# irmen/synthesizer

Hardware: AMD Instinct MI355X
Metric: Msamples/sec mixed to stereo bus, 1024-voice additive @48kHz (higher is better)
Workload: dtype f64

## Files before the change

### synthesizer_amd/csrc/osc_bank.hip

```cpp
#include "osc_host.hpp"
#include <new>
#include <stdlib.h>
#include <math.h>

namespace {

__global__ void k_prepare(BankPtrs B, uint32_t first, uint32_t nvoices, uint64_t start, uint32_t nframes,
                          VoiceLaunch* __restrict__ out, VoiceFM* __restrict__ out_fm) {
    uint32_t vi = blockIdx.x * blockDim.x + threadIdx.x;
    PrepInfo info;
    if (vi < nvoices) prepare_voice(B, first, vi, start, nframes, out, out_fm, info);
}

__global__ __launch_bounds__(64) void k_prepare_chunks(BankPtrs B, LaunchSet S, uint32_t nvoices, uint64_t start, uint32_t nframes) {
    prepare_chunk(B, S, blockIdx.x, nvoices, start, nframes);
}

__global__ __launch_bounds__(64) void k_prepare_segments(BankPtrs B, LaunchSet base, uint32_t nvoices, uint64_t start, uint32_t nframes,
                                                         uint32_t seg_frames) {
    const uint32_t s = blockIdx.y;
    const uint32_t first = s * seg_frames;
    const uint32_t n = nframes - first < seg_frames ? nframes - first : seg_frames;
    prepare_chunk(B, segment_set(base, s, nvoices), blockIdx.x, nvoices, start + first, n);
}

template <bool SLOPED>
__global__ __launch_bounds__(64) void k_prepare_segments_var(BankPtrs B, LaunchSet base, uint32_t nvoices, uint64_t start) {
    const uint32_t s = blockIdx.y;
    const uint32_t first = B.seg_first[s], n = B.seg_first[s + 1] - first;
    prepare_chunk<SLOPED>(B, segment_set(base, s, nvoices), blockIdx.x, nvoices, start + first, n);
}

__global__ __launch_bounds__(256) void k_prepare_tiles(BankPtrs B, TileSet T, uint32_t nvoices, uint64_t start, uint32_t nframes, uint32_t ntiles,
                                                       LaunchSet recs, uint32_t with_recs) {
    const uint32_t c = T.k0 * T.groups + blockIdx.x;
    if (c < (nvoices + 63) / 64)
        prepare_tiles_wave(B, T, nvoices, start, nframes, ntiles, c, blockIdx.y * 4 + (threadIdx.x >> 6), with_recs ? &recs : nullptr);
}

}

namespace shosc {

int launch_prepare_tiles(hipStream_t st, const BankPtrs& P, const TileSet& T, uint32_t nvoices, uint64_t start, uint32_t nframes, const LaunchSet* recs) {
    const uint32_t ntiles = sh::div_up(nframes, TILE_FRAMES);
    if (T.k1 == T.k0) return SH_OK;
    hipLaunchKernelGGL(k_prepare_tiles, dim3((T.k1 - T.k0) * T.groups, sh::div_up(ntiles, 4 * TILES_PER_WAVE)), dim3(256), 0, st, P, T, nvoices, start, nframes, ntiles,
                       recs ? *recs : LaunchSet(), recs ? 1u : 0u);
    SH_CHECK_LAUNCH("k_prepare_tiles");
    return SH_OK;
}

int grow_tile_set(sh::Pooled& block, TileSet& T, uint32_t& carved_tiles, uint32_t ntiles, uint32_t nvoices, uint32_t groups, uint32_t range_chunks, hipStream_t st) {
    const uint32_t mask_k = tile_mask_k(nvoices, groups);
    if (block.ptr && T.recs == (TileRec*)block.ptr && T.groups == groups && T.mask_k == mask_k && carved_tiles == ntiles && T.rec_chunks >= range_chunks) return SH_OK;
    uint32_t rec_chunks = ((range_chunks + range_chunks / 4 + 8) + 7) & ~7u;
    const uint32_t all_chunks = (nvoices + 63) / 64 + groups;
    if (rec_chunks > all_chunks) rec_chunks = all_chunks;
    if (rec_chunks < range_chunks) rec_chunks = range_chunks;
    const size_t slots = (size_t)rec_chunks * 64;
    const size_t b_recs = sizeof(TileRec) * ntiles * slots, b_mask = ((sizeof(uint64_t) * ntiles * groups * mask_k) + 255) & ~(size_t)255;
    int rc = sh::grow_pooled(block, b_recs + 2 * b_mask);
    if (rc) return rc;
    carved_tiles = ntiles;
    char* p = (char*)block.ptr;
    T.recs = (TileRec*)p; p += b_recs;
    T.lean = (uint64_t*)p; p += b_mask;
    T.gen = (uint64_t*)p;
    T.groups = groups;
    T.mask_k = mask_k;
    T.k0 = 0;
    T.k1 = 0;
    T.rec_chunks = rec_chunks;
    if (((nvoices + 63) / 64) != groups * mask_k) SH_HIP(hipMemsetAsync(T.lean, 0, 2 * b_mask, st));
    return SH_OK;
}

LaunchSet launch_set(const sh_bank* b, int k) {
    LaunchSet s;
    s.launch = b->d_launch_buf[k];
    s.fm = b->d_launch_fm_buf[k];
    s.fast = b->d_fast_buf[k];
    s.gen_idx = b->d_gen_idx_buf[k];
    s.counts = b->d_counts_buf[k];
    return s;
}

BankPtrs ptrs(const sh_bank* b) {
    BankPtrs p;
    p.voices = b->d_voices;
    p.segs = b->d_segs;
    p.coefs = b->d_coefs;
    p.partials = b->d_partials;
    p.hint = b->d_hint;
    p.lfo_hint = b->d_hint + b->nvoices;
    p.seg_rot = b->d_seg_rot;
    p.lfo_rot = b->d_lfo_rot;
    p.rows = b->launch_rows;
    p.row_stride = b->launch_row_stride;
    p.fm_row = b->d_fm_row;
    p.pwm_row = b->d_pwm_row;
    p.nseg = 0;
    for (int k = 0; k <= SEG_MAX; ++k) p.seg_first[k] = 0;
    p.gen_sub = 1;
    p.gen_scratch = nullptr;
    p.tiles = TileSet{nullptr, nullptr, nullptr, 0, 0, 0};
    p.next_tiles = p.tiles;
    p.next_tile_wgs = 0;
    p.next_ntiles = 0;
    p.polys = b->d_polys;
    p.chunk_span = b->d_chunk_span;
    return p;
}

template <typename T>
static int upload_array(T** dst, const T* src, size_t count, hipStream_t st) {
    *dst = nullptr;
    size_t bytes = (count ? count : 1) * sizeof(T);
    SH_HIP(hipMalloc((void**)dst, bytes));
    if (count) SH_HIP(hipMemcpyAsync(*dst, src, count * sizeof(T), hipMemcpyHostToDevice, st));
    return SH_OK;
}

std::vector<sh_bank*>& live_banks() {
    static std::vector<sh_bank*> v;
    return v;
}
// ... 391 lines not shown
```

### synthesizer_amd/csrc/osc_device.hpp

```cpp
#pragma once
#include "common.hpp"
#include "devmath.hpp"
#include "renderplan.hpp"
#include <type_traits>

namespace shosc {


constexpr uint32_t TILE_MAX_PIECES = 3;
struct alignas(64) TileRec {
    double t0, dt;
    double rc, rs;
    double ea0, ea1, eb0, eb1;
    double GL, GR;
    double tb[2], db[2];
    uint16_t split[2];
    uint16_t npieces;
    uint16_t corner;
    double pad_;
};
constexpr uint32_t TILE_WALK_PIECES = 16;
static_assert(sizeof(TileRec) == TILE_REC_BYTES && sizeof(TileRec) == 128 && offsetof(TileRec, GL) == 64 && offsetof(TileRec, tb) == 80 && offsetof(TileRec, split) == 112, "TileRec layout");
__device__ __forceinline__ double readlane_f64(double v, uint32_t src) {
    union { double d; int u[2]; } a, b;
    a.d = v;
    b.u[0] = __builtin_amdgcn_readlane(a.u[0], (int)src);
    b.u[1] = __builtin_amdgcn_readlane(a.u[1], (int)src);
    return b.d;
}
__device__ __forceinline__ uint32_t nth_set_bit(uint64_t m, uint32_t p) {
    uint32_t pos = 0;
#pragma unroll
    for (int w = 32; w >= 1; w >>= 1) {
        const uint64_t low = m & ((1ull << w) - 1ull);
        const uint32_t cnt = (uint32_t)__popcll(low);
        if (p >= cnt) { p -= cnt; m >>= w; pos += (uint32_t)w; } else { m = low; }
    }
    return pos;
}
struct TileTheta {
    double   lane_d, t0, dt, tb0, tb1, db0, db1;
    uint32_t lane, s1, s2;
    __device__ __forceinline__ double operator()(int j) const {
        const uint32_t i = lane + (uint32_t)j * 64u;
        const double dd = lane_d + (double)(j * 64);
        double t = fma(dd, dt, t0);
        if (i >= s1) t = fma(dd - (double)s1, db0, tb0);
        if (i >= s2) t = fma(dd - (double)s2, db1, tb1);
        return t;
    }
};
struct TileSet {
    TileRec*  recs;
    uint64_t* lean;
    uint64_t* gen;
    uint32_t  groups, mask_k;
    uint32_t  k0, k1;
    uint32_t  rec_chunks;
};
__host__ __device__ __forceinline__ uint32_t tile_mask_k(uint32_t nvoices, uint32_t groups) {
    const uint32_t nchunks = (nvoices + 63) / 64;
    return ((nchunks + groups - 1) / groups + 7) & ~7u;
}

struct BankPtrs {
    const sh_voice*   voices;
    const sh_segment* segs;
    const double*     coefs;
    const sh_partial* partials;
    uint32_t*         hint;
    uint32_t*         lfo_hint;
    const double2*    seg_rot;
    const double2*    lfo_rot;
    const double*     rows;
    size_t            row_stride;
    const int32_t*    fm_row;
    const int32_t*    pwm_row;
    uint32_t          nseg;
    uint32_t          seg_first[SEG_MAX + 1];
    uint32_t          gen_sub;
    double2*          gen_scratch;
    TileSet           tiles;
    const double*     polys;
    const uint64_t*   chunk_span;
    TileSet           next_tiles;
    uint32_t          next_tile_wgs, next_ntiles;
};

#define SH_CONST_AS __attribute__((address_space(4)))
template <typename T>
__device__ __forceinline__ const T SH_CONST_AS* as_const(const T* p) {
#pragma clang diagnostic push
#pragma clang diagnostic ignored "-Wold-style-cast"
    return (const T SH_CONST_AS*)p;
#pragma clang diagnostic pop
}

constexpr uint32_t FL_KIND = 0xF, FL_FM_SHIFT = 4, FL_FM = 0x30, FL_DENSE = 0x40, FL_ENV_UNIFORM = 0x80,
                   FL_POLY = 0x100, FL_FOLDED = 0x200, FL_FLIP = 0x400, FL_SILENT = 0x800, FL_ONSET = 0x1000;
constexpr uint32_t NO_TAIL = 0xFFFFFFFFu;
constexpr int NXP = 12;

struct alignas(16) VoiceLaunch {
    double   t_base, dt;
    uint32_t remain;
    uint32_t flags;
    const double* harm;
    double   amplitude, bias;
    double   gain_l, gain_r;
    double   g0u, slu;
    uint32_t harm_cnt;
// ... 1144 lines not shown
            }
            is_gen = !is_lean && !is_walk;
            if (is_walk) {
                rec_ea0 = wa0; rec_ea1 = wa1; rec_eb0 = wb0; rec_eb1 = wb1;
                rec_corner = w_corner;
            }
            if (is_lean) {
                rec_t0 = fma(dn0 - (double)p_n0, p_dt, p_t0);
                rec_extra = extra;
#pragma unroll
                for (uint32_t k = 0; k < 2; ++k) rec_split[k] = k < extra ? (uint16_t)((long long)starts[k] - n0) : (uint16_t)0xFFFFu;
            }
        }
        any_general = any_general || is_gen;
        if (sounds) { any_sound = true; last_piece = wb + r; }
        const uint64_t ml = __ballot(is_lean || is_walk), mg = __ballot(is_gen);
        const uint64_t mh = __ballot((is_lean || is_walk) && rec_kind == LEAN_HARM), mm = __ballot((is_lean || is_walk) && rec_kind == LEAN_FM);
        const uint32_t n_harm = (uint32_t)__popcll(mh), n_fm = (uint32_t)__popcll(mm);
        if (is_lean || is_walk) {
            const uint64_t below = (1ull << lane) - 1ull;
            const uint32_t pos = rec_kind == LEAN_HARM ? (uint32_t)__popcll(mh & below)
                               : rec_kind == LEAN_FM ? n_harm + (uint32_t)__popcll(mm & below)
                               : n_harm + n_fm + (uint32_t)__popcll(ml & ~mh & ~mm & below);
            TileRec* __restrict__ q = T.recs + (size_t)t * slots + (c - T.k0 * T.groups) * 64 + pos;
            const uint32_t corner = (rec_corner > 0 && rec_corner < TILE_FRAMES && !(rec_ea0 == rec_eb0 && rec_ea1 == rec_eb1)) ? rec_corner : 0u;
            if (!corner) { rec_eb0 = rec_ea0; rec_eb1 = rec_ea1; }
            double2* __restrict__ q2 = reinterpret_cast<double2*>(q);
            q2[0] = make_double2(rec_t0, win_pick<double>(w_dt, r, 0.0));
            double lfo_angle = 0.0;
            if (rec_kind == LEAN_FM)
                lfo_angle = lnp ? fma(dn0 - (double)ltab[2 * lp].n0 - 0.5, ltab[2 * lp].dt, ltab[2 * lp].t0) : fma(dn0 - 0.5, v.lfo_d, v.lfo_a);
            q2[1] = rec_kind == LEAN_FM ? make_double2(dn0, lfo_angle) : rot;
            q2[2] = make_double2(rec_ea0, rec_ea1);
            q2[3] = make_double2(rec_eb0, rec_eb1);
            q2[4] = make_double2(amp * bgl, amp * bgr);
            union { uint64_t u; double d; } walk_bits;
            walk_bits.u = (uint64_t)(off + wb + r) | ((uint64_t)(off + cnt) << 32);
            q2[5] = is_walk ? make_double2(dn0, walk_bits.d)
                            : make_double2(rec_extra > 0 ? win_pick<double>(w_t0, r + 1, 0.0) : 0.0, rec_extra > 1 ? win_pick<double>(w_t0, r + 2, 0.0) : 0.0);
            q2[6] = make_double2(rec_extra > 0 ? win_pick<double>(w_dt, r + 1, 0.0) : 0.0, rec_extra > 1 ? win_pick<double>(w_dt, r + 2, 0.0) : 0.0);
            union { uint16_t h[4]; double d; } tail;
            tail.h[0] = rec_split[0]; tail.h[1] = rec_split[1]; tail.h[2] = is_walk ? (uint16_t)0 : (uint16_t)(1 + rec_extra); tail.h[3] = (uint16_t)corner;
            union { uint32_t u[2]; double d; } kind_bits;
            kind_bits.u[0] = rec_kind | (rec_kind == LEAN_FM ? ((lnp ? off_c + 2 * lp : 0xFFFFFFu) << 8) : 0u);
            kind_bits.u[1] = lane | (lfo_split_rel << 8);
            q2[7] = make_double2(tail.d, kind_bits.d);
        }
        if (lane == 0) {
            const size_t at = ((size_t)t * T.groups + c % T.groups) * T.mask_k + c / T.groups;
            T.lean[at] = (uint64_t)(uint32_t)__popcll(ml) | ((uint64_t)n_harm << 32) | ((uint64_t)n_fm << 40);
            T.gen[at] = mg;
        }
    }
    if (recs) {
        if (valid && any_general) {
            PrepInfo info;
            prepare_voice<false>(B, 0u, vi, start, nframes, recs->launch, recs->fm, info);
        } else if (valid && any_sound) {
            B.hint[vi] = last_piece;
        }
        if (run == 0 && lane == 0) {
            recs->counts[4 * c] = 0; recs->counts[4 * c + 1] = 0; recs->counts[4 * c + 2] = 0; recs->counts[4 * c + 3] = 0;
        }
    }
}


}
```

### synthesizer_amd/csrc/osc_host.hpp

```cpp
#pragma once
#include "osc_device.hpp"
#include <vector>
#include <algorithm>

using namespace shosc;

struct sh_bank : shr::Facts {
    sh_voice*   d_voices = nullptr;
    sh_segment* d_segs = nullptr;
    double*     d_coefs = nullptr;
    sh_partial* d_partials = nullptr;
    static constexpr int NSETS = shosc::NSETS;
    VoiceLaunch* d_launch_buf[NSETS] = {};
    VoiceFM*    d_launch_fm_buf[NSETS] = {};
    FastRec*    d_fast_buf[NSETS] = {};
    uint32_t*   d_gen_idx_buf[NSETS] = {};
    uint32_t*   d_counts_buf[NSETS] = {};
    uint32_t*   d_hint = nullptr;
    static constexpr uint32_t SELF_TILES = shosc::SELF_TILES;
    uint32_t*   d_self() const { return d_hint + 2 * (size_t)nvoices; }
    bool        run_active = false;
    uint64_t    run_next_start = 0;
    uint32_t    run_nframes = 0, run_groups = 0, run_tile = 0, run_count = 0;
    sh::PendingCombine pending[2];
    int         npending = 0;
    sh::Pooled  parts[4];
    sh::Pooled  seg_block[2];
    LaunchSet   seg_set[2] = {};
    uint32_t    seg_cap[2] = {0, 0};
    sh::Pooled  seg_scratch[2];
    static constexpr int NTILESETS = 4;
    sh::Pooled  tile_block[NTILESETS];
    TileSet     tile_set[NTILESETS] = {};
    uint32_t    tile_carved[NTILESETS] = {0, 0, 0, 0};
    using TileSpec = shr::TileSetSpec;
    TileSpec    tile_spec[NTILESETS];
    uint32_t    tile_count = 0;
    struct Range { const char* lo; const char* hi; };
    Range       last_direct[3] = {};
    bool        overlaps_last_direct(const void* p, size_t bytes) const {
        const char* lo = (const char*)p;
        for (const Range& r : last_direct) if (r.lo && lo < r.hi && r.lo < lo + bytes) return true;
        return false;
    }
    int32_t*    d_fm_row = nullptr;
    int32_t*    d_pwm_row = nullptr;
    int32_t     fm_row_max = -1;
    bool        needs_rows = false;
    const double* launch_rows = nullptr;
    size_t      launch_row_stride = 0;
    sh::Pooled  gen_block;
    LaunchSet   gen_set = {};
    uint32_t    gen_segs = 0;
    double2*    d_seg_rot = nullptr;
    uint64_t*   d_chunk_span = nullptr;
    double*     d_polys = nullptr;
    double2*    d_lfo_rot = nullptr;
    VoiceLaunch* d_launch = nullptr;
    VoiceFM*    d_launch_fm = nullptr;
    int         cur = 0;
    int         last_target = -1;
    using Spec = shr::SetSpec;
    Spec        spec[NSETS];
    void        void_specs() { for (auto& q : spec) q.valid = false; last_target = -1; }
    bool        last_tiled = false;
    uint32_t    last_groups = 0;
    float2*     d_gains = nullptr;
    uint32_t    nsegs = 0, ncoefs = 0, npartials = 0;
    std::vector<sh_voice> h_voices;
};

namespace shosc {
LaunchSet launch_set(const sh_bank* b, int k);
BankPtrs ptrs(const sh_bank* b);
std::vector<sh_bank*>& live_banks();
const shm::sc_pair* trig_table();
int prepare_single(sh_bank* b, uint32_t first, uint32_t count, uint64_t start, uint32_t nframes);
int acquire_records(sh_bank* b, uint64_t start, uint32_t nframes, hipStream_t launch_stream, bool in_run, bool accept_sparse = false, bool* deferred = nullptr);
int prepare_chunks_now(sh_bank* b, uint64_t start, uint32_t nframes, hipStream_t st);
int bank_check_plain(const sh_bank* b, const char* who);
int grow_segment_sets(sh::Pooled& block, LaunchSet& g, uint32_t& cap, uint32_t nseg, uint32_t nvoices);
int launch_prepare_tiles(hipStream_t st, const BankPtrs& P, const TileSet& T, uint32_t nvoices, uint64_t start, uint32_t nframes, const LaunchSet* recs = nullptr);
int grow_tile_set(sh::Pooled& block, TileSet& T, uint32_t& carved_tiles, uint32_t ntiles, uint32_t nvoices, uint32_t groups, uint32_t range_chunks, hipStream_t st);
int launch_prepare_segments(hipStream_t st, const BankPtrs& P, const LaunchSet& base, uint32_t nvoices, uint32_t nseg, uint64_t start,
                            uint32_t nframes, uint32_t seg_frames);
int launch_prepare_segments_var(hipStream_t st, bool sloped, const BankPtrs& P, const LaunchSet& base, uint32_t nvoices, uint32_t nseg, uint64_t start);
int fold_bank(sh_bank* b);
int join_aux();
}
```

### synthesizer_amd/csrc/osc_render.hip

```cpp
#include "osc_host.hpp"
#include "osc_render_kernels.hpp"
#include "renderplan.hpp"
#include <stdlib.h>


namespace {

struct WriteRec { const char* lo; const char* hi; const sh_bank* owner; uint8_t streams; };
std::vector<WriteRec>& bank_writes() {
    static std::vector<WriteRec> v;
    return v;
}
bool overlaps_writes(const sh_bank* b, bool own, uint8_t streams, const void* p, size_t bytes) {
    if (!p) return false;
    const char* lo = (const char*)p;
    for (const WriteRec& r : bank_writes())
        if ((r.owner == b) == own && (!own || (r.streams & streams)) && lo < r.hi && r.lo < lo + bytes) return true;
    return false;
}
void note_write(const sh_bank* b, const void* p, size_t bytes, uint8_t stream_bit) {
    if (!p) return;
    const char* lo = (const char*)p;
    for (WriteRec& r : bank_writes())
        if (r.owner == b && r.lo == lo) { if (lo + bytes > r.hi) r.hi = lo + bytes; r.streams |= stream_bit; return; }
// ... 78 lines not shown
            b->seg_cap[k] = 0;
        }
        release_pooled(b->gen_block);
        b->gen_segs = 0;
        for (int k = 0; k < sh_bank::NTILESETS; ++k) {
            release_pooled(b->tile_block[k]);
            b->tile_carved[k] = 0;
            b->tile_spec[k].valid = false;
        }
    }
}
}

struct RenderLaunch {
    sh_bank* b;
    hipStream_t st;
    shr::Call call;
    const shr::Shape& S;
    uint64_t next_start;
    uint32_t prep_wgs;
    bool use_aux;
    bool records_deferred;
    bool self_prepare;
    bool alone;
    LaunchSet cur, next;
    BusOut out;
    double2* parts;
    FoldIn fold;
    uint32_t* gen_valid;
    LaunchArgs args(const BankPtrs& P, const LaunchSet& set) const {
        return LaunchArgs{P, trig_table(), b->nvoices, S.vpg, set, call.start, call.nframes, self_prepare ? 1u : 0u, alone ? 1u : 0u};
    }
    NextArgs next_args(const LaunchSet& nx, uint32_t wgs) const { return NextArgs{nx, next_start, wgs}; }
};
static dim3 dim(shr::Grid g) { return dim3(g.x, g.y); }

static int launch_tiled(const RenderLaunch& L) {
    sh_bank* b = L.b;
    hipStream_t st = L.st;
    const shr::Shape& S = L.S;
    const shr::TiledGrids G = shr::tiled_grids(*b, S, L.call, L.next.launch != nullptr);
    int rc = SH_OK;
    const int ks = (int)(b->tile_count % sh_bank::NTILESETS);
    TileSet& T = b->tile_set[ks];
    sh_bank::TileSpec& sp = b->tile_spec[ks];
    BankPtrs P = ptrs(b);
    sh::counters().tiled_launches += 1;
    const bool predicted = shr::holds(sp, L.call, S.groups);
    if (predicted) sh::counters().tiled_predicted += 1;
    if (!predicted) {
        rc = grow_tile_set(b->tile_block[ks], T, b->tile_carved[ks], G.ntiles, b->nvoices, S.groups, (G.k1 - G.k0) * S.groups, st);
        if (rc) return rc;
        T.k0 = G.k0; T.k1 = G.k1;
        P.tiles = T;
        const LaunchSet own = launch_set(b, b->cur);
        rc = launch_prepare_tiles(st, P, T, b->nvoices, L.call.start, L.call.nframes, L.records_deferred ? &own : nullptr);
        if (rc) return rc;
    } else if (L.records_deferred) {
        rc = prepare_chunks_now(b, L.call.start, L.call.nframes, st);
        if (rc) return rc;
    }
    sp.valid = false;
    if (L.next.launch) {
        const int k2 = (int)((b->tile_count + 2) % sh_bank::NTILESETS);
        TileSet& T2 = b->tile_set[k2];
        rc = grow_tile_set(b->tile_block[k2], T2, b->tile_carved[k2], G.ntiles, b->nvoices, S.groups, (G.nk1 - G.nk0) * S.groups, st);
        if (rc) return rc;
        T2.k0 = G.nk0; T2.k1 = G.nk1;
        P.next_tiles = T2;
        P.next_ntiles = G.ntiles;
        P.next_tile_wgs = G.next_tile_wgs;
        b->tile_spec[k2] = sh_bank::TileSpec{true, L.next_start, L.call.nframes, S.groups};
    }
    P.tiles = T;
    const LaunchArgs A = L.args(P, L.cur);
    LaunchSet nx = L.next;
    if (!G.next_in_kernel) nx.launch = nullptr;
    const NextArgs N = L.next_args(nx, G.behind);
    if (G.merged) {
        if (b->tile_waveforms) hipLaunchKernelGGL((k_render_tiles<4, 8, 3, true, true>), dim(G.tiles), dim3(256), 0, st, A, N, L.fold, L.parts, L.gen_valid);
        else hipLaunchKernelGGL((k_render_tiles<4, 8, 3, false, true>), dim(G.tiles), dim3(256), 0, st, A, N, L.fold, L.parts, L.gen_valid);
    } else {
        if (b->tile_waveforms) hipLaunchKernelGGL((k_render_tiles<4, 8, 3, true, false>), dim(G.tiles), dim3(256), 0, st, A, N, L.fold, L.parts, L.gen_valid);
        else hipLaunchKernelGGL((k_render_tiles<4, 8, 4, false, false>), dim(G.tiles), dim3(256), 0, st, A, N, L.fold, L.parts, L.gen_valid);
    }
    SH_CHECK_LAUNCH("k_render_tiles");
    if (!G.merged) {
        hipLaunchKernelGGL((k_render_general<4, 4, 4, GEN_TILES>), dim3(G.general.x), dim3(256), 0, st, A, L.parts, L.gen_valid);
        SH_CHECK_LAUNCH("k_render_general(tiles)");
    }
    b->tile_count += 1;
    return SH_OK;
}

static int launch_segmented(const RenderLaunch& L) {
    sh_bank* b = L.b;
    hipStream_t st = L.st;
    const shr::Shape& S = L.S;
    const shr::SegmentedGrids G = shr::segmented_grids(S, L.prep_wgs);
    sh::counters().segmented_launches += 1;
    const int ks = L.use_aux ? 1 : 0;
    LaunchSet& g = b->seg_set[ks];
    int rc = grow_segment_sets(b->seg_block[ks], g, b->seg_cap[ks], S.nseg, b->nvoices);
    if (rc) return rc;
    BankPtrs P = ptrs(b);
    P.nseg = S.nseg;
    for (uint32_t k = 0; k <= S.nseg; ++k) P.seg_first[k] = S.seg_first[k];
    rc = launch_prepare_segments_var(st, true, P, g, b->nvoices, S.nseg, L.call.start);
    if (rc) return rc;
    rc = sh::grow_pooled(b->seg_scratch[ks], G.scratch_bytes);
    if (rc) return rc;
    P.gen_sub = G.SUB;
    P.gen_scratch = (double2*)b->seg_scratch[ks].ptr;
    const LaunchArgs A = L.args(P, g);
    const NextArgs N = L.next_args(L.next, L.prep_wgs);
    rc = launch_render_lean(S.lean_var, S.lean_kind, true, dim(G.lean), st, A, N, L.fold, L.parts);
    if (rc) return rc;
    SH_HIP(hipMemsetAsync(L.gen_valid, 1, G.valid_bytes, st));
    hipLaunchKernelGGL((k_render_general<16, 4, 1, GEN_SEG>), dim(G.general), dim3(1024), 0, st, A, L.parts, L.gen_valid);
    SH_CHECK_LAUNCH("k_render_general(segments)");
    hipLaunchKernelGGL(k_seg_combine, dim(G.combine), dim3(256), 0, st, (const double2*)b->seg_scratch[ks].ptr, G.SUB, G.n0,
// ... 268 lines not shown
```

### synthesizer_amd/csrc/osc_render_kernels.hpp

```cpp
#pragma once
#include "osc_device.hpp"
#include <type_traits>

namespace shosc {
struct BusOut {
    float2*   bus32;
    double2*  bus64;
    uint32_t* pcm16;
    double    pcm_scale;
};
struct FoldIn {
    const double2*  parts;
    const uint32_t* gen_valid;
    BusOut          out;
    uint32_t*       self;
};
struct LaunchArgs {
    BankPtrs              B;
    const shm::sc_pair*   trig_g;
    uint32_t              nvoices, voices_per_group;
    LaunchSet             cur;
    uint64_t              start;
    uint32_t              nframes;
    uint32_t              self_prepare;
// ... 551 lines not shown
        uint32_t p = first;
        if constexpr (KINDS == LEAN_K_ALL) {
            const uint32_t runs = as_const(T.set.counts)[4 * c + 3];
            const uint32_t end_harm = runs & 0xFFu, end_fm = end_harm + ((runs >> 8) & 0xFFu);
            for (; p < end_harm; p += WAVES, q += WAVES) entry(std::integral_constant<int, LEAN_K_HARM>{}, q, p);
            for (; p < end_fm; p += WAVES, q += WAVES) entry(std::integral_constant<int, LEAN_K_FM>{}, q, p);
            for (; p < nfast; p += WAVES, q += WAVES) entry(std::integral_constant<int, LEAN_K_REST>{}, q, p);
        } else {
            const uint32_t span = (T.c1 - T.c0) * 64u;
            for (; p < nfast; p += WAVES, q += WAVES) {
                if (T.alone) {
                    const uint32_t at8 = ((c - T.c0) * 64u + p) * 8u;
                    if (at8 < 4 * span) __builtin_amdgcn_s_setprio(3);
                    else if (at8 < 6 * span) __builtin_amdgcn_s_setprio(2);
                    else if (at8 < 7 * span) __builtin_amdgcn_s_setprio(1);
                    else __builtin_amdgcn_s_setprio(0);
                }
                entry(std::integral_constant<int, KINDS>{}, q, p);
            }
        }
        first = p - nfast;
    }
}

template <int WAVES, int FPL>
__device__ __forceinline__ void general_lists(const LaunchArgs& A, const TileCtx& T, uint32_t& first, uint32_t nsub, const uint32_t (&i)[FPL],
                                              const double (&di)[FPL], TrigTab trig, double (&accl)[FPL], double (&accr)[FPL]) {
    for (uint32_t c = T.c0; c < T.c1; ++c) {
        const uint32_t ngen = as_const(T.set.counts)[4 * c + 1];
        const uint32_t SH_CONST_AS* idx = as_const(T.set.gen_idx) + c * 64;
        const uint32_t step = WAVES * nsub;
        uint32_t p = first;
        uint32_t vi_next = p < ngen ? idx[p] : 0u;
        for (; p < ngen; p += step) {
            const uint32_t vi = vi_next;
            vi_next = p + step < ngen ? idx[p + step] : 0u;
            const VoiceRegs r = load_record(as_const(T.set.launch) + vi);
            general_voice<FPL>(r, T.set.fm + vi, A.B, A.B.voices + vi, T.st0, T.tile0, T.nfr, i, di, trig, accl, accr);
        }
        first = p - ngen;
    }
}

__device__ __forceinline__ uint32_t general_count(const uint32_t* counts, uint32_t c0, uint32_t c1) {
    uint32_t total = 0;
    for (uint32_t c = c0; c < c1; ++c) total += as_const(counts)[4 * c + 1];
    return total;
}

enum { TILE_RUN_HARM = 0, TILE_RUN_FM = 1, TILE_RUN_REST = 2 };
template <int WAVES, int FPL, bool WAVEFORMS>
__device__ __forceinline__ void tiles_lean(const BankPtrs& B, const TileCtx& T, TrigTab trig, double (&accl)[FPL], double (&accr)[FPL]) {
    static_assert(64 * FPL == TILE_FRAMES, "the lean kernel's tile is the tile of the classification");
    const uint32_t lane = T.lane, ngroups = T.ngroups, tile_index = T.tile_index;
    const size_t slots = (size_t)B.tiles.rec_chunks * 64;
    const TileRec SH_CONST_AS* trow = as_const(B.tiles.recs) + (size_t)tile_index * slots;
    const uint32_t kw = B.tiles.k1 - B.tiles.k0, nmask = ngroups * kw, stride = ngroups * WAVES;
    const uint64_t* __restrict__ lrow = B.tiles.lean + (size_t)tile_index * (ngroups * B.tiles.mask_k);
    uint32_t firstp = __builtin_amdgcn_readfirstlane(T.grp * WAVES + T.wave);
    for (uint32_t base = 0; base < nmask; base += 64) {
        const uint32_t mi = base + lane;
        const uint64_t mymask = mi < nmask ? lrow[(mi / kw) * B.tiles.mask_k + B.tiles.k0 + mi % kw] : 0ull;
        const uint64_t have0 = __ballot(mymask != 0ull);
        uint64_t have = ((uint64_t)(uint32_t)__builtin_amdgcn_readfirstlane((int)(uint32_t)(have0 >> 32)) << 32) |
                        (uint64_t)(uint32_t)__builtin_amdgcn_readfirstlane((int)(uint32_t)have0);
        while (have) {
            const uint32_t src = (uint32_t)__builtin_ctzll(have);
            have &= have - 1;
            const uint64_t cmask = ((uint64_t)(uint32_t)__builtin_amdgcn_readlane((int)(uint32_t)(mymask >> 32), (int)src) << 32) |
                                   (uint64_t)(uint32_t)__builtin_amdgcn_readlane((int)(uint32_t)mymask, (int)src);
            const uint32_t npairs = (uint32_t)cmask;
            const uint32_t idx = base + src;
            const uint32_t c = idx / kw + (B.tiles.k0 + idx % kw) * ngroups;
            auto pair = [&](auto cls_, const TileRec SH_CONST_AS* q) __attribute__((always_inline)) {
                constexpr int CLS = decltype(cls_)::value;
                const double t0 = q->t0, dt = q->dt, rc = q->rc, rs = q->rs, ea0 = q->ea0, ea1 = q->ea1, GL = q->GL, GR = q->GR;
                const uint32_t pc = *reinterpret_cast<const uint32_t SH_CONST_AS*>(&q->npieces);
                uint32_t lane_again = lane;
                asm volatile("" : "+v"(lane_again));
                const double lane_d = (double)lane_again;
                const uint32_t vword = *reinterpret_cast<const uint32_t SH_CONST_AS*>(reinterpret_cast<const char SH_CONST_AS*>(&q->pad_) + 4);
                const uint32_t vbit = vword & 0xFFu;
                const double SH_CONST_AS* pp = as_const(B.polys) + (size_t)(c * 64 + vbit) * 16;
                double poly[16];
#pragma unroll
                for (int v_ = 0; v_ < 16; ++v_) poly[v_] = pp[v_];
                asm volatile("" :: "s"(t0), "s"(dt), "s"(rc), "s"(rs), "s"(ea0), "s"(ea1), "s"(GL), "s"(GR), "s"(pc),
                             "s"(poly[0]), "s"(poly[1]), "s"(poly[2]), "s"(poly[3]), "s"(poly[4]), "s"(poly[5]),
                             "s"(poly[6]), "s"(poly[7]), "s"(poly[8]), "s"(poly[9]), "s"(poly[10]), "s"(poly[11]), "s"(poly[12]),
                             "s"(poly[13]), "s"(poly[14]), "s"(poly[15]));
                const LaneTheta none{0.0, 0.0, 0.0, 0.0, 0.0, 0.0, 0.0, 0.0, 0.0, 0u, 0u, false};
                if constexpr (CLS != TILE_RUN_HARM) {
                    double lfo_d = 0.0, lfo_K = 0.0, lfo_C0 = 0.0, lrc = 1.0, lrs = 0.0, lfo2_a = 0.0, lfo2_d = 0.0, lfo2_K = 0.0, lfo2_C0 = 0.0;
                    uint32_t lfo_split = 0;
                    if constexpr (CLS == TILE_RUN_FM) {
                        const uint32_t lfo_idx = *reinterpret_cast<const uint32_t SH_CONST_AS*>(&q->pad_) >> 8;
                        const sh_segment SH_CONST_AS* lpc_ = as_const(B.segs) + (lfo_idx != 0xFFFFFFu ? lfo_idx : 0u);
                        if (lfo_idx != 0xFFFFFFu) {
                            const sh_segment SH_CONST_AS* lpc = lpc_;
                            const double2 SH_CONST_AS* lro = as_const(B.seg_rot) + lfo_idx;
                            lfo_d = lpc[0].dt; lfo_K = lpc[1].t0; lfo_C0 = lpc[1].dt; lrc = lro->x; lrs = lro->y;
                        } else {
                            lfo_d = poly[4]; lfo_K = poly[5]; lfo_C0 = poly[6]; lrc = poly[8]; lrs = poly[9];
                        }
                        lfo_split = vword >> 8;
                        if (lfo_split) {
                            lfo2_d = lpc_[2].dt; lfo2_a = fma(-(double)lfo_split - 0.5, lfo2_d, lpc_[2].t0); lfo2_K = lpc_[3].t0; lfo2_C0 = lpc_[3].dt;
                        }
                        if (pc == 1u && lfo_split == 0u) {
                            double sn[FPL];
                            const double t_first = fma(lane_d, dt, t0), t_step = 64.0 * dt;
                            lean_fm_frames<FPL, false, true>(poly, rs, rc, lfo_d, lfo_K, lfo_C0, lrc, lrs, lane_d, none, t_first, t_step, trig, sn);
                            double gl_e = GL, gr_e = GR;
                            if (ea1 == 0.0) {
                                gl_e = GL * ea0;
                                gr_e = GR * ea0;
                            } else {
#pragma unroll
                                for (int j = 0; j < FPL; ++j) sn[j] = sn[j] * fma(lane_d + (double)(j * 64), ea1, ea0);
                            }
#pragma unroll
                            for (int j = 0; j < FPL; ++j) {
                                accl[j] = fma(gl_e, sn[j], accl[j]);
                                accr[j] = fma(gr_e, sn[j], accr[j]);
                            }
                            return;
                        }
                    }
                    const uint32_t wkind = *reinterpret_cast<const uint32_t SH_CONST_AS*>(&q->pad_) & 0xFFu;
                    {
                        const double eb0 = q->eb0, eb1 = q->eb1, ci = (double)(pc >> 16);
                        double th[FPL], on = 0.0;
                        if ((pc & 0xFFFFu) == 0u) {
                            const double dn0 = q->tb[0];
                            const uint64_t wbits = *reinterpret_cast<const uint64_t SH_CONST_AS*>(&q->tb[1]);
                            const uint32_t seg_first = (uint32_t)wbits, seg_end = (uint32_t)(wbits >> 32);
// ... 75 lines not shown
                    s1 = fma(s0, rc, c0s * rs);
                    c1s = fma(c0s, rc, -(s0 * rs));
                    lean_harm_values<FPL>(s0, c0s, s1, c1s, rc + rc, false, none, trig, poly, w);
#pragma unroll
                    for (int j = 0; j < FPL; ++j) w[j] = w[j] * tile_envelope(lane_d + (double)(j * 64), ci, ea0, ea1, eb0, eb1);
                } else if ((pc & 0xFFFFu) == 0u) {
                    const double eb0 = q->eb0, eb1 = q->eb1, dn0 = q->tb[0], ci = (double)(pc >> 16);
                    const uint64_t wbits = *reinterpret_cast<const uint64_t SH_CONST_AS*>(&q->tb[1]);
                    const uint32_t seg_first = (uint32_t)wbits, seg_end = (uint32_t)(wbits >> 32);
                    const uint32_t kidx = seg_first + (lane & (TILE_WALK_PIECES - 1));
                    const bool have_piece = lane < TILE_WALK_PIECES && kidx < seg_end;
                    const sh_segment* sp = B.segs + (have_piece ? kidx : seg_first);
                    const uint64_t pn0 = sp->n0;
                    const double pt0 = sp->t0, pdt = sp->dt;
                    const double prel = (double)(long long)pn0 - dn0;
                    const uint32_t npc = (uint32_t)__popcll(__ballot(have_piece && prel < (double)TILE_FRAMES));
                    double th[FPL];
#pragma unroll
                    for (int j = 0; j < FPL; ++j) th[j] = 0.0;
                    for (uint32_t k = 0; k < npc; ++k) {
                        const double rk = readlane_f64(prel, k), tk = readlane_f64(pt0, k), dk = readlane_f64(pdt, k);
#pragma unroll
                        for (int j = 0; j < FPL; ++j) {
                            const double x = lane_d + (double)(j * 64);
                            th[j] = x >= rk ? fma(x - rk, dk, tk) : th[j];
                        }
                    }
#pragma unroll
                    for (int j = 0; j < FPL; ++j) {
                        double sj, cj;
                        shm::sincos_tab(th[j], trig, sj, cj);
                        double pj = fma(poly[0], cj, poly[1]);
#pragma unroll
                        for (int u = 2; u < 16; ++u) pj = fma(pj, cj, poly[u]);
                        w[j] = (pj * sj) * tile_envelope(lane_d + (double)(j * 64), ci, ea0, ea1, eb0, eb1);
                    }
                } else {
                    const double eb0 = q->eb0, eb1 = q->eb1, ci = (double)(pc >> 16);
                    const TileTheta theta{lane_d, t0, dt, q->tb[0], q->tb[1], q->db[0], q->db[1], lane, q->split[0], q->split[1]};
                    double s0, c0s, s1, c1s;
                    shm::sincos_tab(theta(0), trig, s0, c0s);
                    shm::sincos_tab(theta(1), trig, s1, c1s);
                    lean_harm_values<FPL>(s0, c0s, s1, c1s, 0.0, true, theta, trig, poly, w);
#pragma unroll
                    for (int j = 0; j < FPL; ++j) w[j] = w[j] * tile_envelope(lane_d + (double)(j * 64), ci, ea0, ea1, eb0, eb1);
                }
#pragma unroll
                for (int j = 0; j < FPL; ++j) {
                    accl[j] = fma(gl_e, w[j], accl[j]);
                    accr[j] = fma(gr_e, w[j], accr[j]);
                }
                }
            };
            const TileRec SH_CONST_AS* q = trow + (c - B.tiles.k0 * ngroups) * 64 + firstp;
            uint32_t p = firstp;
            if constexpr (WAVEFORMS) {
                const uint32_t end_harm = (uint32_t)(cmask >> 32) & 0xFFu, end_fm = end_harm + ((uint32_t)(cmask >> 40) & 0xFFu);
                for (; p < end_harm; p += stride, q += stride) pair(std::integral_constant<int, TILE_RUN_HARM>{}, q);
                for (; p < end_fm; p += stride, q += stride) pair(std::integral_constant<int, TILE_RUN_FM>{}, q);
                for (; p < npairs; p += stride, q += stride) pair(std::integral_constant<int, TILE_RUN_REST>{}, q);
            } else {
                for (; p < npairs; p += stride, q += stride) pair(std::integral_constant<int, TILE_RUN_HARM>{}, q);
            }
            firstp = __builtin_amdgcn_readfirstlane(p - npairs);
        }
    }
}

template <int WAVES>
__device__ __forceinline__ bool tile_has_general(const BankPtrs& B, uint32_t class_tile) {
    const uint32_t kw = B.tiles.k1 - B.tiles.k0, nmask = B.tiles.groups * kw;
    const uint64_t* __restrict__ grow = B.tiles.gen + (size_t)class_tile * (B.tiles.groups * B.tiles.mask_k);
    bool any = false;
    for (uint32_t base = 0; base < nmask; base += 64) {
        const uint32_t mi = base + (threadIdx.x & 63);
        const uint64_t mine = mi < nmask ? grow[(mi / kw) * B.tiles.mask_k + B.tiles.k0 + mi % kw] : 0ull;
        any = any || __ballot(mine != 0ull) != 0ull;
    }
    return any;
}
template <int WAVES, int FPL>
__device__ __forceinline__ void tiles_general(const LaunchArgs& A, const TileCtx& T, uint32_t gen_part, const uint32_t (&i)[FPL], const double (&di)[FPL],
                                              TrigTab trig, double (&accl)[FPL], double (&accr)[FPL]) {
    const BankPtrs& B = A.B;
    const uint32_t kw = B.tiles.k1 - B.tiles.k0, nmask = B.tiles.groups * kw;
    const uint64_t* __restrict__ grow = B.tiles.gen + (size_t)(T.tile0 / TILE_FRAMES) * (B.tiles.groups * B.tiles.mask_k);
    uint32_t ord = 0;
    for (uint32_t base = 0; base < nmask; base += 64) {
        const uint32_t mi = base + T.lane;
        const uint64_t mine = mi < nmask ? grow[(mi / kw) * B.tiles.mask_k + B.tiles.k0 + mi % kw] : 0ull;
        uint64_t have = __ballot(mine != 0ull);
        while (have) {
            const uint32_t src = (uint32_t)__builtin_ctzll(have);
            have &= have - 1;
            uint64_t m = ((uint64_t)(uint32_t)__builtin_amdgcn_readlane((int)(uint32_t)(mine >> 32), (int)src) << 32) |
                         (uint64_t)(uint32_t)__builtin_amdgcn_readlane((int)(uint32_t)mine, (int)src);
            const uint32_t idx = base + src;
            const uint32_t c = idx / kw + (B.tiles.k0 + idx % kw) * B.tiles.groups;
            while (m) {
                const uint32_t bit = (uint32_t)__builtin_ctzll(m);
                m &= m - 1;
                if ((ord++ % (uint32_t)(WAVES * GEN_SPLIT)) != T.wave * GEN_SPLIT + gen_part) continue;
                const uint32_t vi = c * 64 + bit;
                const VoiceRegs r = load_record(as_const(T.set.launch) + vi);
                general_voice<FPL>(r, T.set.fm + vi, B, B.voices + vi, T.st0, T.tile0, T.nfr, i, di, trig, accl, accr);
            }
        }
    }
}
template <int WAVES, int FPL>
__device__ __forceinline__ void zero_tile(double2* __restrict__ plane, uint32_t tile_first, uint32_t nfr) {
    for (uint32_t f = threadIdx.x; f < 64 * FPL; f += WAVES * 64) {
        const uint32_t raw = tile_first + f;
        if (raw < nfr) plane[raw] = make_double2(0.0, 0.0);
    }
}

template <int FPL>
__device__ __forceinline__ void clear_acc(double (&accl)[FPL], double (&accr)[FPL]) {
#pragma unroll
    for (int j = 0; j < FPL; ++j) {
        accl[j] = 0.0;
        accr[j] = 0.0;
// ... 211 lines not shown
```

### synthesizer_amd/csrc/renderplan.hpp

```cpp
#pragma once
#include "genplan.hpp"

namespace shosc {
enum { COMBINED_DIRECT = 0, COMBINED_LEAN_HARM = 1, COMBINED_LEAN_ALL = 2 };
enum { LEAN_K_HARM = 0, LEAN_K_ALL = 1, LEAN_K_FM = 2, LEAN_K_REST = 3 };
constexpr uint32_t TILE_FRAMES = 512;
constexpr uint32_t TILE_REC_BYTES = 128;
constexpr uint32_t GEN_SPLIT = 2;
#ifndef SH_TPW
#define SH_TPW 3
#endif
constexpr uint32_t TILES_PER_WAVE = SH_TPW;
constexpr uint32_t SELF_TILES = 16384;
constexpr int      NSETS = 4;
}

namespace shr {
using namespace shosc;
using shg::div_up;

struct Facts : shg::BankFacts {
    uint32_t    lean_fmsine_candidates = 0;
    bool        has_onsets = false;
    bool        own_envelopes = false;
// ... 82 lines not shown
    S.mode = mode; S.var = var; S.W = W; S.F = F;
    S.tile_candidate = tile_candidate;
    S.tiles = tiles; S.groups = groups; S.vpg = vpg; S.nchunks = div_up(B.nvoices, 64);
    S.split = split;
    S.kind = PLAIN;
    if (split && tile_candidate && var == 484) {
        const ChunkRange r = sounding_chunks(B, start, nframes);
        S.c_lo = r.lo; S.c_hi = r.hi;
        const uint64_t range = r.hi > r.lo ? (uint64_t)(r.hi - r.lo) + 2 * groups : 0;
        if ((uint64_t)div_up(nframes, TILE_FRAMES) * range * 64 * TILE_REC_BYTES <= ((uint64_t)1 << 31)) S.kind = TILED;
    }
    if (S.kind != TILED && split && (var == 484 || var == 4163) && B.all_lean && !K.no_seg && !c.reads_rows && !quiet()) {
        S.nseg = shg::plan_segments(B, start, nframes, (uint64_t)(64 * F), ~0ull, true, S.seg_first);
        if (S.nseg < 2 || S.seg_first[S.nseg] != nframes) S.nseg = 0;
        if (S.nseg) S.kind = SEGMENTED;
    }
    S.with_general = split && !quiet();
    S.lean_kind = mode == COMBINED_LEAN_HARM ? LEAN_K_HARM : (S.kind == PLAIN && fm_only ? LEAN_K_FM : LEAN_K_ALL);
    S.lean_var = S.kind == SEGMENTED ? 484 : var;
    S.combined = S.kind == PLAIN && !split;
    S.parts_bytes = groups <= 1 ? 0 : split ? 2 * (size_t)groups * nframes * 16 + (size_t)groups * sizeof(uint32_t) : (size_t)groups * nframes * 16;
    S.may_pipeline = !K.no_speculation && !K.no_overlap;
    S.direct = groups == 1;
    S.pipelined = groups > 1 || (S.may_pipeline && !K.no_small_pipeline);
    return S;
}

struct RunView { bool active; uint32_t nframes, groups, tile; uint64_t next_start; };
inline bool continues_run(const RunView& R, const Shape& S, const Call& c) {
    return S.pipelined && R.active && R.nframes == c.nframes && R.groups == S.groups && R.tile == (uint32_t)(64 * S.F) && R.next_start == c.start;
}
struct SetSpec { bool valid = false; uint64_t start = 0; uint32_t nframes = 0; bool sparse = false; };
inline int next_record_set(const SetSpec (&spec)[NSETS], int cur, int prev_cur, int last_target, bool cont, const Call& c, const Knobs& K) {
    if (K.no_speculation) return -1;
    for (int s = 0; s < NSETS; ++s) {
        const bool holds_between = spec[s].valid && spec[s].start == c.start + c.nframes && spec[s].nframes == c.nframes;
        if (s != cur && !(cont && (s == prev_cur || s == last_target)) && !holds_between) return s;
    }
    return -1;
}
struct TileSetSpec { bool valid = false; uint64_t start = 0; uint32_t nframes = 0, groups = 0; };
inline bool holds(const TileSetSpec& sp, const Call& c, uint32_t groups) { return sp.valid && sp.start == c.start && sp.nframes == c.nframes && sp.groups == groups; }
inline bool plain_split(const Shape& S, const Knobs& K) { return S.split && S.kind == PLAIN && K.self != 0; }
inline bool may_self_prepare(const Shape& S, const Knobs& K) { return plain_split(S, K) && K.self != 2; }
inline bool self_fold(const Shape& S, const Knobs& K, bool cont, int npending) {
    return plain_split(S, K) && K.self != 3 && S.groups > 1 && !cont && npending == 0 && !S.with_general && S.tiles <= SELF_TILES;
}
inline bool stands_alone(bool cont, const Knobs& K) { return !cont && !K.no_ladder; }
inline uint32_t prepare_workgroups(const Shape& S, int target) { return target >= 0 ? S.nchunks : 0u; }

struct Grid { uint32_t x, y; };
inline Grid behind_groups(const Shape& S, uint32_t tiles, uint32_t behind) { return Grid{tiles, S.groups + div_up(behind, tiles)}; }

struct TiledGrids {
    uint32_t ntiles;
    uint32_t k0, k1;
    uint32_t nk0, nk1;
    uint32_t next_tile_wgs;
    bool     merged;
    uint32_t behind;
    bool     next_in_kernel;
    Grid     tiles, general;
};
inline void mask_slots(ChunkRange r, uint32_t groups, uint32_t& k0, uint32_t& k1) {
    k0 = r.hi ? r.lo / groups : 0u;
    k1 = r.hi ? div_up(r.hi, groups) : 0u;
}
inline TiledGrids tiled_grids(const Facts& B, const Shape& S, const Call& c, bool has_next) {
    TiledGrids G{};
    G.ntiles = div_up(c.nframes, TILE_FRAMES);
    mask_slots(ChunkRange{S.c_lo, S.c_hi}, S.groups, G.k0, G.k1);
    if (has_next) {
        mask_slots(sounding_chunks(B, c.start + 2 * (uint64_t)c.nframes, c.nframes), S.groups, G.nk0, G.nk1);
        uint32_t in_range = (G.nk1 - G.nk0) * S.groups;
        if (G.nk1 * S.groups > S.nchunks) in_range -= G.nk1 * S.groups - S.nchunks;
        G.next_tile_wgs = in_range * div_up(div_up(G.ntiles, TILES_PER_WAVE), 4);
    }
    G.merged = S.tiles <= 16;
    G.behind = G.merged ? S.tiles * GEN_SPLIT + G.next_tile_wgs : G.next_tile_wgs;
    G.next_in_kernel = has_next && (G.merged || G.behind);
    G.tiles = behind_groups(S, S.tiles, G.behind);
    G.general = Grid{div_up(c.nframes, 256) * GEN_SPLIT, 1};
    return G;
}

struct SegmentedGrids {
    uint32_t tiles_lean, tiles_gen;
    uint32_t SUB, n0;
    size_t   scratch_bytes, valid_bytes;
    Grid     lean, general, combine;
};
inline SegmentedGrids segmented_grids(const Shape& S, uint32_t prep_wgs) {
    SegmentedGrids G{};
    for (uint32_t k = 0; k < S.nseg; ++k) {
        G.tiles_lean += div_up(S.seg_first[k + 1] - S.seg_first[k], 64 * 8);
        G.tiles_gen += div_up(S.seg_first[k + 1] - S.seg_first[k], 64 * 4);
    }
    G.SUB = 4;
    G.n0 = S.seg_first[1];
    G.scratch_bytes = (size_t)S.groups * G.SUB * G.n0 * 16;
    G.valid_bytes = (size_t)S.groups * sizeof(uint32_t);
    G.lean = behind_groups(S, G.tiles_lean, prep_wgs);
    G.general = Grid{G.tiles_gen + (G.SUB - 1) * div_up(G.n0, 64 * 4), S.groups};
    G.combine = Grid{div_up(G.n0, 256), S.groups};
    return G;
}
// ... 8 lines not shown
```

Before: 1.380 million.

## Add global any-general stamp to skip per-tile general scans; hoist lean-kernel addressing

The tile-prepare kernel now writes a per-launch stamp into a single global word whenever any wave sees a general voice. The render's tile_has_general checks that word first and returns false early, which avoids scanning the per-tile gen masks when no general voices exist. Separately, the lean tile loop moves index arithmetic out of the inner loop: chunk ids are computed per lane and fetched with readlane, scalar bases come from readfirstlane, and record and polynomial pointers are built from precomputed bases. The stamp adds a small allocation and memset, and it relies on prepare running before render on the same stream.

```diff
diff --git a/synthesizer_amd/csrc/osc_bank.hip b/synthesizer_amd/csrc/osc_bank.hip
--- a/synthesizer_amd/csrc/osc_bank.hip
+++ b/synthesizer_amd/csrc/osc_bank.hip
@@ -60,19 +60,22 @@
     if (rec_chunks < range_chunks) rec_chunks = range_chunks;
     const size_t slots = (size_t)rec_chunks * 64;
     const size_t b_recs = sizeof(TileRec) * ntiles * slots, b_mask = ((sizeof(uint64_t) * ntiles * groups * mask_k) + 255) & ~(size_t)255;
-    int rc = sh::grow_pooled(block, b_recs + 2 * b_mask);
+    int rc = sh::grow_pooled(block, b_recs + 2 * b_mask + 256);
     if (rc) return rc;
     carved_tiles = ntiles;
     char* p = (char*)block.ptr;
     T.recs = (TileRec*)p; p += b_recs;
     T.lean = (uint64_t*)p; p += b_mask;
-    T.gen = (uint64_t*)p;
+    T.gen = (uint64_t*)p; p += b_mask;
+    T.any_gen = (uint64_t*)p;
+    T.stamp = 0;
     T.groups = groups;
     T.mask_k = mask_k;
     T.k0 = 0;
     T.k1 = 0;
     T.rec_chunks = rec_chunks;
     if (((nvoices + 63) / 64) != groups * mask_k) SH_HIP(hipMemsetAsync(T.lean, 0, 2 * b_mask, st));
+    SH_HIP(hipMemsetAsync(T.any_gen, 0, sizeof(uint64_t), st));
     return SH_OK;
 }
 
diff --git a/synthesizer_amd/csrc/osc_device.hpp b/synthesizer_amd/csrc/osc_device.hpp
--- a/synthesizer_amd/csrc/osc_device.hpp
+++ b/synthesizer_amd/csrc/osc_device.hpp
@@ -57,6 +57,8 @@
     uint32_t  groups, mask_k;
     uint32_t  k0, k1;
     uint32_t  rec_chunks;
+    uint64_t* any_gen;
+    uint64_t  stamp;
 };
 __host__ __device__ __forceinline__ uint32_t tile_mask_k(uint32_t nvoices, uint32_t groups) {
     const uint32_t nchunks = (nvoices + 63) / 64;
@@ -1307,6 +1309,7 @@
             T.gen[at] = mg;
         }
     }
+    if (__ballot(any_general) != 0ull && lane == 0) *T.any_gen = T.stamp;
     if (recs) {
         if (valid && any_general) {
             PrepInfo info;
diff --git a/synthesizer_amd/csrc/osc_host.hpp b/synthesizer_amd/csrc/osc_host.hpp
--- a/synthesizer_amd/csrc/osc_host.hpp
+++ b/synthesizer_amd/csrc/osc_host.hpp
@@ -36,6 +36,7 @@
     using TileSpec = shr::TileSetSpec;
     TileSpec    tile_spec[NTILESETS];
     uint32_t    tile_count = 0;
+    uint64_t    tile_stamp = 0;
     struct Range { const char* lo; const char* hi; };
     Range       last_direct[3] = {};
     bool        overlaps_last_direct(const void* p, size_t bytes) const {
diff --git a/synthesizer_amd/csrc/osc_render.hip b/synthesizer_amd/csrc/osc_render.hip
--- a/synthesizer_amd/csrc/osc_render.hip
+++ b/synthesizer_amd/csrc/osc_render.hip
@@ -154,6 +154,7 @@
         rc = grow_tile_set(b->tile_block[ks], T, b->tile_carved[ks], G.ntiles, b->nvoices, S.groups, (G.k1 - G.k0) * S.groups, st);
         if (rc) return rc;
         T.k0 = G.k0; T.k1 = G.k1;
+        T.stamp = shr::next_tile_stamp(b->tile_stamp);
         P.tiles = T;
         const LaunchSet own = launch_set(b, b->cur);
         rc = launch_prepare_tiles(st, P, T, b->nvoices, L.call.start, L.call.nframes, L.records_deferred ? &own : nullptr);
@@ -169,6 +170,7 @@
         rc = grow_tile_set(b->tile_block[k2], T2, b->tile_carved[k2], G.ntiles, b->nvoices, S.groups, (G.nk1 - G.nk0) * S.groups, st);
         if (rc) return rc;
         T2.k0 = G.nk0; T2.k1 = G.nk1;
+        T2.stamp = shr::next_tile_stamp(b->tile_stamp);
         P.next_tiles = T2;
         P.next_ntiles = G.ntiles;
         P.next_tile_wgs = G.next_tile_wgs;
diff --git a/synthesizer_amd/csrc/osc_render_kernels.hpp b/synthesizer_amd/csrc/osc_render_kernels.hpp
--- a/synthesizer_amd/csrc/osc_render_kernels.hpp
+++ b/synthesizer_amd/csrc/osc_render_kernels.hpp
@@ -627,15 +627,18 @@
 template <int WAVES, int FPL, bool WAVEFORMS>
 __device__ __forceinline__ void tiles_lean(const BankPtrs& B, const TileCtx& T, TrigTab trig, double (&accl)[FPL], double (&accr)[FPL]) {
     static_assert(64 * FPL == TILE_FRAMES, "the lean kernel's tile is the tile of the classification");
-    const uint32_t lane = T.lane, ngroups = T.ngroups, tile_index = T.tile_index;
+    const uint32_t lane = T.lane, ngroups = (uint32_t)__builtin_amdgcn_readfirstlane((int)T.ngroups);
+    const uint32_t tile_index = (uint32_t)__builtin_amdgcn_readfirstlane((int)T.tile_index);
     const size_t slots = (size_t)B.tiles.rec_chunks * 64;
-    const TileRec SH_CONST_AS* trow = as_const(B.tiles.recs) + (size_t)tile_index * slots;
-    const uint32_t kw = B.tiles.k1 - B.tiles.k0, nmask = ngroups * kw, stride = ngroups * WAVES;
+    const uint32_t k0 = B.tiles.k0, kw = B.tiles.k1 - k0, nmask = ngroups * kw, stride = ngroups * WAVES;
     const uint64_t* __restrict__ lrow = B.tiles.lean + (size_t)tile_index * (ngroups * B.tiles.mask_k);
+    const uint64_t rec_base = reinterpret_cast<uint64_t>(B.tiles.recs) + ((uint64_t)tile_index * slots - (uint64_t)(k0 * ngroups) * 64u) * sizeof(TileRec);
+    const uint64_t poly_base = reinterpret_cast<uint64_t>(B.polys);
     uint32_t firstp = __builtin_amdgcn_readfirstlane(T.grp * WAVES + T.wave);
     for (uint32_t base = 0; base < nmask; base += 64) {
-        const uint32_t mi = base + lane;
-        const uint64_t mymask = mi < nmask ? lrow[(mi / kw) * B.tiles.mask_k + B.tiles.k0 + mi % kw] : 0ull;
+        const uint32_t mi = base + lane, mg = mi / kw, mk = mi - mg * kw;
+        const uint64_t mymask = mi < nmask ? lrow[mg * B.tiles.mask_k + k0 + mk] : 0ull;
+        const uint32_t mychunk = mg + (k0 + mk) * ngroups;
         const uint64_t have0 = __ballot(mymask != 0ull);
         uint64_t have = ((uint64_t)(uint32_t)__builtin_amdgcn_readfirstlane((int)(uint32_t)(have0 >> 32)) << 32) |
                         (uint64_t)(uint32_t)__builtin_amdgcn_readfirstlane((int)(uint32_t)have0);
@@ -645,8 +648,8 @@
             const uint64_t cmask = ((uint64_t)(uint32_t)__builtin_amdgcn_readlane((int)(uint32_t)(mymask >> 32), (int)src) << 32) |
                                    (uint64_t)(uint32_t)__builtin_amdgcn_readlane((int)(uint32_t)mymask, (int)src);
             const uint32_t npairs = (uint32_t)cmask;
-            const uint32_t idx = base + src;
-            const uint32_t c = idx / kw + (B.tiles.k0 + idx % kw) * ngroups;
+            const uint32_t c = (uint32_t)__builtin_amdgcn_readlane((int)mychunk, (int)src);
+            const double SH_CONST_AS* pchunk = reinterpret_cast<const double SH_CONST_AS*>(poly_base + (uint64_t)c * (64u * 16u * sizeof(double)));
             auto pair = [&](auto cls_, const TileRec SH_CONST_AS* q) __attribute__((always_inline)) {
                 constexpr int CLS = decltype(cls_)::value;
                 const double t0 = q->t0, dt = q->dt, rc = q->rc, rs = q->rs, ea0 = q->ea0, ea1 = q->ea1, GL = q->GL, GR = q->GR;
@@ -656,7 +659,7 @@
                 const double lane_d = (double)lane_again;
                 const uint32_t vword = *reinterpret_cast<const uint32_t SH_CONST_AS*>(reinterpret_cast<const char SH_CONST_AS*>(&q->pad_) + 4);
                 const uint32_t vbit = vword & 0xFFu;
-                const double SH_CONST_AS* pp = as_const(B.polys) + (size_t)(c * 64 + vbit) * 16;
+                const double SH_CONST_AS* pp = pchunk + vbit * 16u;
                 double poly[16];
 #pragma unroll
                 for (int v_ = 0; v_ < 16; ++v_) poly[v_] = pp[v_];
@@ -838,7 +841,7 @@
                 }
                 }
             };
-            const TileRec SH_CONST_AS* q = trow + (c - B.tiles.k0 * ngroups) * 64 + firstp;
+            const TileRec SH_CONST_AS* q = reinterpret_cast<const TileRec SH_CONST_AS*>(rec_base + ((uint64_t)c * 64u + firstp) * sizeof(TileRec));
             uint32_t p = firstp;
             if constexpr (WAVEFORMS) {
                 const uint32_t end_harm = (uint32_t)(cmask >> 32) & 0xFFu, end_fm = end_harm + ((uint32_t)(cmask >> 40) & 0xFFu);
@@ -855,6 +858,7 @@
 
 template <int WAVES>
 __device__ __forceinline__ bool tile_has_general(const BankPtrs& B, uint32_t class_tile) {
+    if (as_const(B.tiles.any_gen)[0] != B.tiles.stamp) return false;
     const uint32_t kw = B.tiles.k1 - B.tiles.k0, nmask = B.tiles.groups * kw;
     const uint64_t* __restrict__ grow = B.tiles.gen + (size_t)class_tile * (B.tiles.groups * B.tiles.mask_k);
     bool any = false;
diff --git a/synthesizer_amd/csrc/renderplan.hpp b/synthesizer_amd/csrc/renderplan.hpp
--- a/synthesizer_amd/csrc/renderplan.hpp
+++ b/synthesizer_amd/csrc/renderplan.hpp
@@ -158,6 +158,8 @@
 struct Grid { uint32_t x, y; };
 inline Grid behind_groups(const Shape& S, uint32_t tiles, uint32_t behind) { return Grid{tiles, S.groups + div_up(behind, tiles)}; }
 
+inline uint64_t next_tile_stamp(uint64_t& last) { return ++last; }
+
 struct TiledGrids {
     uint32_t ntiles;
     uint32_t k0, k1;
```

Result: no change. 1.381 million (median of 3 runs) (+0.1%).
